# mcmilk/7-Zip-zstd

Hardware: NVIDIA H100
Metric: zstd-L3 encode+decode throughput (higher is better)
Workload: dtype u8

## Files before the change

7-zip-zstd_b200/csrc/zstd_enc_find.cu:

```cuda
#include "b2z_device.cuh"
#include "b2z_kernels.h"

namespace b2z {

#define B2Z_FIND_BAR_TURN(g) (1u + (g))
#define B2Z_FIND_BAR_GRP(g)  (8u + (g))

__device__ __forceinline__ void turn_inputs_ready(uint32_t* slot, uint32_t iL, uint32_t iS, uint32_t mineL, uint32_t mineS, uint32_t flags) {
#ifndef B2Z_CUEMU
    const uint32_t mix = iL ^ (iS << 8) ^ mineL ^ (mineS >> 3) ^ flags;
    asm volatile("st.volatile.shared.u32 [%0], %1;" :: "r"((uint32_t)__cvta_generic_to_shared(slot)), "r"(mix) : "memory");
#else
    (void)slot; (void)iL; (void)iS; (void)mineL; (void)mineS; (void)flags;
#endif
}

struct B16 { uint32_t x0, x1, x2, x3; };
static_assert(B2Z_CAP == 16, "stage F compares four 32-bit words");
template <bool GUARD>
__device__ __forceinline__ B16 ld16(const uint32_t* __restrict__ w4, uint32_t o, uint32_t nW4) {
    const uint32_t a = o >> 2, sh = (o & 3u) * 8u;
    uint32_t t0, t1, t2, t3, t4;
    if (GUARD) {
        t0 = a < nW4 ? __ldg(w4 + a) : 0u; t1 = a + 1u < nW4 ? __ldg(w4 + a + 1u) : 0u; t2 = a + 2u < nW4 ? __ldg(w4 + a + 2u) : 0u;
        t3 = a + 3u < nW4 ? __ldg(w4 + a + 3u) : 0u; t4 = a + 4u < nW4 ? __ldg(w4 + a + 4u) : 0u;
    } else { t0 = __ldg(w4 + a); t1 = __ldg(w4 + a + 1u); t2 = __ldg(w4 + a + 2u); t3 = __ldg(w4 + a + 3u); t4 = __ldg(w4 + a + 4u); }
    B16 r; r.x0 = __funnelshift_r(t0, t1, sh); r.x1 = __funnelshift_r(t1, t2, sh); r.x2 = __funnelshift_r(t2, t3, sh); r.x3 = __funnelshift_r(t3, t4, sh);
    return r;
}
__device__ __forceinline__ uint32_t prefix16(const B16& a, const B16& b) {
    const uint32_t d0 = a.x0 ^ b.x0, d1 = a.x1 ^ b.x1, d2 = a.x2 ^ b.x2, d3 = a.x3 ^ b.x3;
    const uint32_t z = d0 ? d0 : (d1 ? d1 : (d2 ? d2 : d3));
    const uint32_t base = d0 ? 0u : (d1 ? 4u : (d2 ? 8u : 12u));
    return z ? base + ((uint32_t)(__ffs((int)z) - 1) >> 3) : 16u;
}

struct FindCtx {
    uint32_t* smem; uint32_t* TL; uint32_t* TS; uint32_t tableWords, HL, HS, tagBits, tagMask, W, tid, grp, tg, nextGrp;
};

template <int WPG, int G, int MODE, bool GUARD>
__device__ __forceinline__ void find_frame(const FindCtx& c, const uint32_t* __restrict__ w4, uint32_t n, uint32_t* __restrict__ out) {
    constexpr uint32_t CH = WPG * 32u;
    constexpr bool FAST = MODE == 1, STEP = MODE == 2;
    const uint32_t nW4 = (n + 3u) >> 2;
    const uint32_t HL = c.HL, HS = c.HS, tagBits = c.tagBits, tagMask = c.tagMask;
    const uint32_t nChunks = (n + CH - 1u) / CH, nIter = (nChunks + G - 1u) / G;
    B16 vNext = ld16<true>(w4, c.grp * CH + c.tg, nW4);
    for (uint32_t it = 0; it < nIter; it++) {
        const uint32_t p = (it * G + c.grp) * CH + c.tg;
        const B16 own = vNext;
        const uint64_t v = (uint64_t)own.x0 | ((uint64_t)own.x1 << 32);
        const bool hashable = p + 8u <= n;
        const uint64_t hl = v * B2Z_PRIME8, hs = (v << 24) * B2Z_PRIME5;
        const uint32_t iL = (uint32_t)(hl >> (64u - HL)), iS = (uint32_t)(hs >> (64u - HS));
        const uint32_t tL = (uint32_t)(hl >> (64u - HL - tagBits)) & tagMask, tS = (uint32_t)(hs >> (64u - HS - tagBits)) & tagMask;
        const uint32_t mineL = ((p + 1u) << tagBits) | tL, mineS = ((p + 1u) << tagBits) | tS;
        uint32_t* const aL = c.TL + iL; uint32_t* const aS = c.TS + iS;
        uint32_t lowL = 0, lowS = 0;
        if (STEP) {
            const uint32_t lane = c.tid & 31u, lt = (1u << lane) - 1u;
            lowL = __match_any_sync(B2Z_FULL, hashable ? iL : (0x80000000u | lane)) & lt;
            lowS = __match_any_sync(B2Z_FULL, hashable ? iS : (0x80000000u | lane)) & lt;
        }
        turn_inputs_ready(c.smem + c.tableWords + c.tid, iL, iS, mineL, mineS, (uint32_t)hashable ^ lowL ^ (lowS << 1));
        bar_sync(B2Z_FIND_BAR_TURN(c.grp), 2u * CH);
        uint32_t eL = 0, eS = 0;
        if (hashable) { if (!FAST) eL = *aL; eS = *aS; }
        if (WPG > 1) bar_sync(B2Z_FIND_BAR_GRP(c.grp), CH); else __syncwarp();
        if (hashable) { if (!FAST) atomicMax(aL, mineL); atomicMax(aS, mineS); }
        bar_arrive(B2Z_FIND_BAR_TURN(c.nextGrp), 2u * CH);
        if (STEP) {
            const uint32_t fromL = __shfl_sync(B2Z_FULL, mineL, lowL ? 31 - __clz((int)lowL) : 0);
            const uint32_t fromS = __shfl_sync(B2Z_FULL, mineS, lowS ? 31 - __clz((int)lowS) : 0);
            if (lowL) eL = fromL;
            if (lowS) eS = fromS;
        }
        vNext = ld16<GUARD>(w4, p + G * CH, nW4);
        uint32_t word = 0;
        if (hashable) {
            const uint32_t segEnd = ((p | (B2Z_SEG - 1u)) + 1u) < n ? ((p | (B2Z_SEG - 1u)) + 1u) : n;
            const uint32_t maxLen = (segEnd - p) < B2Z_CAP ? (segEnd - p) : B2Z_CAP;
            uint32_t lenL = 0, offL = 0, lenS = 0, offS = 0;
            if (eL && (eL & tagMask) == tL) { const uint32_t q = (eL >> tagBits) - 1u; if (p - q <= c.W) { offL = p - q; const uint32_t l = prefix16(ld16<GUARD>(w4, q, nW4), own); lenL = l < maxLen ? l : maxLen; } }
            if (eS && (eS & tagMask) == tS) { const uint32_t q = (eS >> tagBits) - 1u; if (p - q <= c.W && p - q != offL) { offS = p - q; const uint32_t l = prefix16(ld16<GUARD>(w4, q, nW4), own); lenS = l < maxLen ? l : maxLen; } }
            uint32_t len = lenL, off = offL;
            if (lenS > lenL || (lenS == lenL && lenS && offS < offL)) { len = lenS; off = offS; }
            if (len >= B2Z_DP_MINLEN) word = B2Z_CAND(len, off);
        }
        if (p < n) __stcs(out + p, word);
    }
}

template <int WPG, int G, int MODE>
__global__ void __launch_bounds__(WPG * G * 32, 1)
zstd_enc_find_kernel(const uint8_t* __restrict__ src, uint64_t srcSize, EncGeom g, uint32_t* __restrict__ cand,
                     const volatile uint32_t* ready, uint32_t readyShift, uint32_t* __restrict__ errFlag) {
    B2Z_EXTERN_SMEM(uint32_t, smem);
    constexpr uint32_t CH = WPG * 32u, NT = CH * G;
    static_assert(G >= 2 && G <= 7, "named barriers 1..7 and 8..14");
    FindCtx c;
    c.tid = threadIdx.x; c.grp = c.tid / CH; c.tg = c.tid % CH;
    c.HL = g.hashLogL; c.HS = g.hashLogS;
    c.smem = smem;
    c.TL = smem;
    c.TS = smem + (MODE == 1 ? 0u : (1u << c.HL));
    c.tableWords = (MODE == 1 ? 0u : (1u << c.HL)) + (1u << c.HS);
    c.tagBits = 32u - (g.frameLog + 1u); c.tagMask = (1u << c.tagBits) - 1u;
    c.W = g.windowLog >= 32 ? 0xFFFFFFFFu : (1u << g.windowLog);
    c.nextGrp = c.grp + 1u == (uint32_t)G ? 0u : c.grp + 1u;
    const uint64_t nFrames = (srcSize + (1ull << g.frameLog) - 1) >> g.frameLog;
    const uint32_t tid = c.tid;

    if (c.grp == (uint32_t)G - 1u) bar_arrive(B2Z_FIND_BAR_TURN(0), 2u * CH);

    for (uint64_t f = blockIdx.x; f < nFrames; f += gridDim.x) {
        const uint64_t f0 = f << g.frameLog;
        const uint32_t n = enc_frame_bytes(g, srcSize, f);
        const uint32_t* __restrict__ w4 = reinterpret_cast<const uint32_t*>(src + f0);
        uint32_t* __restrict__ out = cand + f0;
        if (ready && n) {
            if (tid == 0) {
                uint32_t spins = 0;
                while (ready[(f0 + n - 1u) >> readyShift] == 0u) { if (++spins > (1u << 22)) { atomicExch(errFlag, 1u); break; } __nanosleep(1000); }
            }
        }
        __syncthreads();
        for (uint32_t i = tid; i < c.tableWords / 4u; i += NT) reinterpret_cast<uint4*>(smem)[i] = make_uint4(0, 0, 0, 0);
        __syncthreads();
        if (srcSize - f0 - n >= 4096u) find_frame<WPG, G, MODE, false>(c, w4, n, out);
        else find_frame<WPG, G, MODE, true>(c, w4, n, out);
    }
    if (c.grp == 0) bar_sync(B2Z_FIND_BAR_TURN(0), 2u * CH);
}

#ifndef B2Z_CUEMU
size_t zstd_enc_find_smem_bytes(const EncGeom& g) {
    return (((g.flags & B2Z_FLAG_FIND_FAST) ? 0 : ((size_t)1 << g.hashLogL)) + ((size_t)1 << g.hashLogS) + 1024u) * 4u;
}

template <int WPG, int G, int MODE>
static cudaError_t launch_find_m(const uint8_t* src, uint64_t srcSize, const EncGeom& g, uint32_t* cand, uint32_t nCtas,
                                 const uint32_t* ready, uint32_t readyShift, uint32_t* errFlag, cudaStream_t st) {
    const size_t smem = zstd_enc_find_smem_bytes(g);
    cudaError_t e = cudaFuncSetAttribute(zstd_enc_find_kernel<WPG, G, MODE>, cudaFuncAttributeMaxDynamicSharedMemorySize, (int)smem);
    if (e != cudaSuccess) return e;
    zstd_enc_find_kernel<WPG, G, MODE><<<nCtas, WPG * G * 32, smem, st>>>(src, srcSize, g, cand, ready, readyShift, errFlag);
    return cudaGetLastError();
}
template <int WPG, int G>
static cudaError_t launch_find_t(const uint8_t* src, uint64_t srcSize, const EncGeom& g, uint32_t* cand, uint32_t nCtas,
                                 const uint32_t* ready, uint32_t readyShift, uint32_t* errFlag, cudaStream_t st) {
    if (g.flags & B2Z_FLAG_FIND_FAST) return launch_find_m<WPG, G, 1>(src, srcSize, g, cand, nCtas, ready, readyShift, errFlag, st);
    if (g.flags & B2Z_FLAG_FIND_STEP) return launch_find_m<WPG, G, 2>(src, srcSize, g, cand, nCtas, ready, readyShift, errFlag, st);
    return launch_find_m<WPG, G, 0>(src, srcSize, g, cand, nCtas, ready, readyShift, errFlag, st);
}

cudaError_t launch_zstd_enc_find(const uint8_t* src, uint64_t srcSize, const EncGeom& g, uint32_t* cand, uint32_t nCtas,
                                 const uint32_t* ready, uint32_t readyShift, uint32_t* errFlag, cudaStream_t st) {
    if (srcSize == 0) return cudaSuccess;
    switch (g.chunkLog) {
    case 5: return launch_find_t<1, 7>(src, srcSize, g, cand, nCtas, ready, readyShift, errFlag, st);
    case 6: return launch_find_t<2, 7>(src, srcSize, g, cand, nCtas, ready, readyShift, errFlag, st);
    case 7: return launch_find_t<4, 7>(src, srcSize, g, cand, nCtas, ready, readyShift, errFlag, st);
    case 8: return launch_find_t<8, 4>(src, srcSize, g, cand, nCtas, ready, readyShift, errFlag, st);
    }
    return cudaErrorInvalidValue;
}
#endif

}
```

Baseline: 28710.

## Streamline find-stage inner loop: 32-bit hashing, branchless candidate selection, strength-reduced addressing

Rewrites the match-finding inner loop to compute only the needed high 32 bits of the 64-bit hash products using 32-bit multiplies. Table reads and atomicMax now run unconditionally, writing 0 for non-hashable positions. Candidate validation and selection become branchless by always loading both candidates and packing length and offset into one comparable key. Loop addresses are strength-reduced, barrier IDs are precomputed, and compile-time-gated clock instrumentation plus a geometry validity check are added. The aim is fewer instructions and less divergence in the latency-bound find kernel, at the cost of extra unconditional loads.

```diff
diff --git a/7-zip-zstd_b200/csrc/zstd_enc_find.cu b/7-zip-zstd_b200/csrc/zstd_enc_find.cu
--- a/7-zip-zstd_b200/csrc/zstd_enc_find.cu
+++ b/7-zip-zstd_b200/csrc/zstd_enc_find.cu
@@ -17,14 +17,17 @@
 
 struct B16 { uint32_t x0, x1, x2, x3; };
 static_assert(B2Z_CAP == 16, "stage F compares four 32-bit words");
+__device__ __forceinline__ B16 ld16p(const uint32_t* __restrict__ w, uint32_t sh) {
+    const uint32_t t0 = __ldg(w), t1 = __ldg(w + 1), t2 = __ldg(w + 2), t3 = __ldg(w + 3), t4 = __ldg(w + 4);
+    B16 r; r.x0 = __funnelshift_r(t0, t1, sh); r.x1 = __funnelshift_r(t1, t2, sh); r.x2 = __funnelshift_r(t2, t3, sh); r.x3 = __funnelshift_r(t3, t4, sh);
+    return r;
+}
 template <bool GUARD>
 __device__ __forceinline__ B16 ld16(const uint32_t* __restrict__ w4, uint32_t o, uint32_t nW4) {
-    const uint32_t a = o >> 2, sh = (o & 3u) * 8u;
-    uint32_t t0, t1, t2, t3, t4;
-    if (GUARD) {
-        t0 = a < nW4 ? __ldg(w4 + a) : 0u; t1 = a + 1u < nW4 ? __ldg(w4 + a + 1u) : 0u; t2 = a + 2u < nW4 ? __ldg(w4 + a + 2u) : 0u;
-        t3 = a + 3u < nW4 ? __ldg(w4 + a + 3u) : 0u; t4 = a + 4u < nW4 ? __ldg(w4 + a + 4u) : 0u;
-    } else { t0 = __ldg(w4 + a); t1 = __ldg(w4 + a + 1u); t2 = __ldg(w4 + a + 2u); t3 = __ldg(w4 + a + 3u); t4 = __ldg(w4 + a + 4u); }
+    const uint32_t a = o >> 2, sh = o * 8u;
+    if (!GUARD) return ld16p(w4 + a, sh);
+    const uint32_t t0 = a < nW4 ? __ldg(w4 + a) : 0u, t1 = a + 1u < nW4 ? __ldg(w4 + a + 1u) : 0u, t2 = a + 2u < nW4 ? __ldg(w4 + a + 2u) : 0u;
+    const uint32_t t3 = a + 3u < nW4 ? __ldg(w4 + a + 3u) : 0u, t4 = a + 4u < nW4 ? __ldg(w4 + a + 4u) : 0u;
     B16 r; r.x0 = __funnelshift_r(t0, t1, sh); r.x1 = __funnelshift_r(t1, t2, sh); r.x2 = __funnelshift_r(t2, t3, sh); r.x3 = __funnelshift_r(t3, t4, sh);
     return r;
 }
@@ -32,30 +35,53 @@
     const uint32_t d0 = a.x0 ^ b.x0, d1 = a.x1 ^ b.x1, d2 = a.x2 ^ b.x2, d3 = a.x3 ^ b.x3;
     const uint32_t z = d0 ? d0 : (d1 ? d1 : (d2 ? d2 : d3));
     const uint32_t base = d0 ? 0u : (d1 ? 4u : (d2 ? 8u : 12u));
-    return z ? base + ((uint32_t)(__ffs((int)z) - 1) >> 3) : 16u;
+    return base + ((uint32_t)(__ffs((int)z) - 1) >> 3);
 }
 
 struct FindCtx {
-    uint32_t* smem; uint32_t* TL; uint32_t* TS; uint32_t tableWords, HL, HS, tagBits, tagMask, W, tid, grp, tg, nextGrp;
+    uint32_t* smem; uint32_t* TL; uint32_t* TS; uint32_t tableWords, HL, HS, tagBits, tagMask, W, tid, grp, tg;
+    uint32_t barTurn, barGrp, barNext;
 };
 
+enum { FC_WAIT, FC_TURN, FC_CAND, FC_WORK, FC_N };
+#ifdef B2Z_F_CLOCKS
+__device__ unsigned long long f_clocks[FC_N + 1];
+#define F_TICK(ph) do { const long long now_ = clock64(); fc[ph] += (unsigned long long)(now_ - fcLast); fcLast = now_; } while (0)
+#else
+#define F_TICK(ph) do { } while (0)
+#endif
+
 template <int WPG, int G, int MODE, bool GUARD>
-__device__ __forceinline__ void find_frame(const FindCtx& c, const uint32_t* __restrict__ w4, uint32_t n, uint32_t* __restrict__ out) {
-    constexpr uint32_t CH = WPG * 32u;
+__device__ __forceinline__ void find_frame(const FindCtx& c, const uint32_t* __restrict__ w4, uint32_t n, uint32_t* __restrict__ out
+#ifdef B2Z_F_CLOCKS
+                                           , unsigned long long* fc, long long& fcLast
+#endif
+                                           ) {
+    constexpr uint32_t CH = WPG * 32u, STEPW = G * CH;
     constexpr bool FAST = MODE == 1, STEP = MODE == 2;
     const uint32_t nW4 = (n + 3u) >> 2;
-    const uint32_t HL = c.HL, HS = c.HS, tagBits = c.tagBits, tagMask = c.tagMask;
+    const uint32_t HL = c.HL, HS = c.HS, tagBits = c.tagBits, W = c.W;
+    uint32_t tagMask = c.tagMask;
+#ifndef B2Z_CUEMU
+    asm("mov.b64 %0, %0;" : "+l"(w4)); asm("mov.b32 %0, %0;" : "+r"(tagMask));
+#endif
+    constexpr uint64_t PL = B2Z_PRIME8, PS = B2Z_PRIME5 << 24;
+    const uint32_t shIL = 32u - HL, shIS = 32u - HS, shTL = 32u - HL - tagBits, shTS = 32u - HS - tagBits;
     const uint32_t nChunks = (n + CH - 1u) / CH, nIter = (nChunks + G - 1u) / G;
-    B16 vNext = ld16<true>(w4, c.grp * CH + c.tg, nW4);
-    for (uint32_t it = 0; it < nIter; it++) {
-        const uint32_t p = (it * G + c.grp) * CH + c.tg;
+    uint32_t p = c.grp * CH + c.tg;
+    B16 vNext = ld16<true>(w4, p, nW4);
+    uint32_t aNext = (p >> 2) + STEPW / 4u;
+    const uint32_t shOwn = p * 8u;
+    uint32_t* __restrict__ o = out + p;
+    for (uint32_t it = 0; it < nIter; it++, p += STEPW, aNext += STEPW / 4u, o += STEPW) {
         const B16 own = vNext;
-        const uint64_t v = (uint64_t)own.x0 | ((uint64_t)own.x1 << 32);
         const bool hashable = p + 8u <= n;
-        const uint64_t hl = v * B2Z_PRIME8, hs = (v << 24) * B2Z_PRIME5;
-        const uint32_t iL = (uint32_t)(hl >> (64u - HL)), iS = (uint32_t)(hs >> (64u - HS));
-        const uint32_t tL = (uint32_t)(hl >> (64u - HL - tagBits)) & tagMask, tS = (uint32_t)(hs >> (64u - HS - tagBits)) & tagMask;
+        const uint32_t hl = (uint32_t)(((uint64_t)own.x0 * (uint32_t)PL) >> 32) + own.x0 * (uint32_t)(PL >> 32) + own.x1 * (uint32_t)PL;
+        const uint32_t hs = (uint32_t)(((uint64_t)own.x0 * (uint32_t)PS) >> 32) + own.x0 * (uint32_t)(PS >> 32) + own.x1 * (uint32_t)PS;
+        const uint32_t iL = hl >> shIL, iS = hs >> shIS;
+        const uint32_t tL = (hl >> shTL) & tagMask, tS = (hs >> shTS) & tagMask;
         const uint32_t mineL = ((p + 1u) << tagBits) | tL, mineS = ((p + 1u) << tagBits) | tS;
+        const uint32_t putL = hashable ? mineL : 0u, putS = hashable ? mineS : 0u;
         uint32_t* const aL = c.TL + iL; uint32_t* const aS = c.TS + iS;
         uint32_t lowL = 0, lowS = 0;
         if (STEP) {
@@ -63,32 +89,44 @@
             lowL = __match_any_sync(B2Z_FULL, hashable ? iL : (0x80000000u | lane)) & lt;
             lowS = __match_any_sync(B2Z_FULL, hashable ? iS : (0x80000000u | lane)) & lt;
         }
-        turn_inputs_ready(c.smem + c.tableWords + c.tid, iL, iS, mineL, mineS, (uint32_t)hashable ^ lowL ^ (lowS << 1));
-        bar_sync(B2Z_FIND_BAR_TURN(c.grp), 2u * CH);
-        uint32_t eL = 0, eS = 0;
-        if (hashable) { if (!FAST) eL = *aL; eS = *aS; }
-        if (WPG > 1) bar_sync(B2Z_FIND_BAR_GRP(c.grp), CH); else __syncwarp();
-        if (hashable) { if (!FAST) atomicMax(aL, mineL); atomicMax(aS, mineS); }
-        bar_arrive(B2Z_FIND_BAR_TURN(c.nextGrp), 2u * CH);
+        turn_inputs_ready(c.smem + c.tableWords + c.tid, iL, iS, putL, putS, c.barNext ^ lowL ^ (lowS << 1));
+        F_TICK(FC_WORK);
+        bar_sync(c.barTurn, 2u * CH);
+        F_TICK(FC_WAIT);
+        uint32_t eL = 0, eS;
+        if (!FAST) eL = *aL;
+        eS = *aS;
+        if (WPG > 1) bar_sync(c.barGrp, CH); else __syncwarp();
+        if (!FAST) atomicMax(aL, putL);
+        atomicMax(aS, putS);
+        bar_arrive(c.barNext, 2u * CH);
+        F_TICK(FC_TURN);
         if (STEP) {
             const uint32_t fromL = __shfl_sync(B2Z_FULL, mineL, lowL ? 31 - __clz((int)lowL) : 0);
             const uint32_t fromS = __shfl_sync(B2Z_FULL, mineS, lowS ? 31 - __clz((int)lowS) : 0);
             if (lowL) eL = fromL;
             if (lowS) eS = fromS;
         }
-        vNext = ld16<GUARD>(w4, p + G * CH, nW4);
+        if (GUARD) vNext = ld16<true>(w4, p + STEPW, nW4);
+        else vNext = ld16p(w4 + aNext, shOwn);
         uint32_t word = 0;
         if (hashable) {
+            const uint32_t offL = p - ((eL >> tagBits) - 1u), offS = p - ((eS >> tagBits) - 1u);
+            const bool okL = !FAST && hashable && eL && (eL & tagMask) == tL && offL <= W;
+            const bool okS = hashable && eS && (eS & tagMask) == tS && offS <= W && !(okL && offS == offL);
+            const B16 cL = ld16<GUARD>(w4, p - (okL ? offL : 0u), nW4);
+            const B16 cS = ld16<GUARD>(w4, p - (okS ? offS : 0u), nW4);
             const uint32_t segEnd = ((p | (B2Z_SEG - 1u)) + 1u) < n ? ((p | (B2Z_SEG - 1u)) + 1u) : n;
             const uint32_t maxLen = (segEnd - p) < B2Z_CAP ? (segEnd - p) : B2Z_CAP;
-            uint32_t lenL = 0, offL = 0, lenS = 0, offS = 0;
-            if (eL && (eL & tagMask) == tL) { const uint32_t q = (eL >> tagBits) - 1u; if (p - q <= c.W) { offL = p - q; const uint32_t l = prefix16(ld16<GUARD>(w4, q, nW4), own); lenL = l < maxLen ? l : maxLen; } }
-            if (eS && (eS & tagMask) == tS) { const uint32_t q = (eS >> tagBits) - 1u; if (p - q <= c.W && p - q != offL) { offS = p - q; const uint32_t l = prefix16(ld16<GUARD>(w4, q, nW4), own); lenS = l < maxLen ? l : maxLen; } }
-            uint32_t len = lenL, off = offL;
-            if (lenS > lenL || (lenS == lenL && lenS && offS < offL)) { len = lenS; off = offS; }
-            if (len >= B2Z_DP_MINLEN) word = B2Z_CAND(len, off);
-        }
-        if (p < n) __stcs(out + p, word);
+            const uint32_t lL = prefix16(cL, own), lS = prefix16(cS, own);
+            F_TICK(FC_CAND);
+            const uint32_t mL = okL ? maxLen : 0u, mS = okS ? maxLen : 0u;
+            const uint32_t lenL = FAST ? 0u : (lL < mL ? lL : mL), lenS = lS < mS ? lS : mS;
+            const uint32_t kL = (lenL << 24) | (~offL & 0xFFFFFFu), kS = (lenS << 24) | (~offS & 0xFFFFFFu);
+            const uint32_t k = kS > kL ? kS : kL, len = k >> 24;
+            word = len >= B2Z_DP_MINLEN ? B2Z_CAND(len, ~k & 0xFFFFFFu) : 0u;
+        }
+        if (p < n) __stcs(o, word);
     }
 }
 
@@ -108,9 +146,17 @@
     c.tableWords = (MODE == 1 ? 0u : (1u << c.HL)) + (1u << c.HS);
     c.tagBits = 32u - (g.frameLog + 1u); c.tagMask = (1u << c.tagBits) - 1u;
     c.W = g.windowLog >= 32 ? 0xFFFFFFFFu : (1u << g.windowLog);
-    c.nextGrp = c.grp + 1u == (uint32_t)G ? 0u : c.grp + 1u;
+    c.barTurn = B2Z_FIND_BAR_TURN(c.grp); c.barGrp = B2Z_FIND_BAR_GRP(c.grp);
+    c.barNext = B2Z_FIND_BAR_TURN(c.grp + 1u == (uint32_t)G ? 0u : c.grp + 1u);
     const uint64_t nFrames = (srcSize + (1ull << g.frameLog) - 1) >> g.frameLog;
     const uint32_t tid = c.tid;
+#ifdef B2Z_F_CLOCKS
+    unsigned long long fc[FC_N] = {};
+    long long fcLast = clock64();
+#define B2Z_F_CLOCK_ARGS , fc, fcLast
+#else
+#define B2Z_F_CLOCK_ARGS
+#endif
 
     if (c.grp == (uint32_t)G - 1u) bar_arrive(B2Z_FIND_BAR_TURN(0), 2u * CH);
 
@@ -128,10 +174,15 @@
         __syncthreads();
         for (uint32_t i = tid; i < c.tableWords / 4u; i += NT) reinterpret_cast<uint4*>(smem)[i] = make_uint4(0, 0, 0, 0);
         __syncthreads();
-        if (srcSize - f0 - n >= 4096u) find_frame<WPG, G, MODE, false>(c, w4, n, out);
-        else find_frame<WPG, G, MODE, true>(c, w4, n, out);
+        F_TICK(FC_WORK);
+        if (srcSize - f0 - n >= 4096u) find_frame<WPG, G, MODE, false>(c, w4, n, out B2Z_F_CLOCK_ARGS);
+        else find_frame<WPG, G, MODE, true>(c, w4, n, out B2Z_F_CLOCK_ARGS);
     }
+#undef B2Z_F_CLOCK_ARGS
     if (c.grp == 0) bar_sync(B2Z_FIND_BAR_TURN(0), 2u * CH);
+#ifdef B2Z_F_CLOCKS
+    if ((tid & 31u) == 0) { for (int p_ = 0; p_ < FC_N; p_++) atomicAdd(&f_clocks[p_], fc[p_]); atomicAdd(&f_clocks[FC_N], 1ull); }
+#endif
 }
 
 #ifndef B2Z_CUEMU
@@ -159,6 +210,8 @@
 cudaError_t launch_zstd_enc_find(const uint8_t* src, uint64_t srcSize, const EncGeom& g, uint32_t* cand, uint32_t nCtas,
                                  const uint32_t* ready, uint32_t readyShift, uint32_t* errFlag, cudaStream_t st) {
     if (srcSize == 0) return cudaSuccess;
+    const uint32_t hashLog = g.hashLogL > g.hashLogS ? g.hashLogL : g.hashLogS;
+    if (g.frameLog < 17 || g.frameLog > B2Z_MAX_FRAMELOG || hashLog + 31u - g.frameLog > 32u) return cudaErrorInvalidValue;
     switch (g.chunkLog) {
     case 5: return launch_find_t<1, 7>(src, srcSize, g, cand, nCtas, ready, readyShift, errFlag, st);
     case 6: return launch_find_t<2, 7>(src, srcSize, g, cand, nCtas, ready, readyShift, errFlag, st);
@@ -167,6 +220,15 @@
     }
     return cudaErrorInvalidValue;
 }
-#endif
-
-}
+
+#ifdef B2Z_F_CLOCKS
+extern "C" int b200z_find_clocks(unsigned long long* out) {
+    static const unsigned long long zero[FC_N + 1] = {};
+    cudaError_t e = cudaMemcpyFromSymbol(out, f_clocks, sizeof(f_clocks));
+    if (e == cudaSuccess) e = cudaMemcpyToSymbol(f_clocks, zero, sizeof(f_clocks));
+    return (int)e;
+}
+#endif
+#endif
+
+}
```

After: 30370 (median of 6 runs). 5.8% higher.
